# steineggerlab/unicore

Measured on AMD Instinct MI355X. Metric: 3Di alignments/sec (cluster path), higher is better.
Workload: dtype u16

## Files before the change

### include/unicore_cluster.h

```cpp
#ifndef UNICORE_CLUSTER_H
#define UNICORE_CLUSTER_H
#include <stddef.h>
#include <stdint.h>
#ifdef __cplusplus
extern "C" {
#endif

#define UC_OK 0
#define UC_ERR_GENERIC 1
#define UC_ERR_ARGS 2
#define UC_ERR_IO 3
#define UC_ERR_DEVICE 4

typedef struct uc_opts {
    uint32_t struct_size;
    int32_t threads;
    int32_t verbosity;
    int32_t device;
    int32_t num_gpus;
    const char *cluster_options;
    const char *data_dir;
} uc_opts;

#define UC_ABI_VERSION 9
// ... 94 lines not shown
int uc_hits_merge(uint32_t n_seqs, int32_t max_seqs, int n_parts, const uint32_t *const *counts,
                  const uc_hit *const *hits, uint32_t *out_counts, uc_hit *out_hits, uint64_t out_capacity,
                  uint64_t *out_n);

int uc_engine_hits_export_dev(const uc_engine *e, uint32_t *d_query, uint32_t *d_target, int32_t *d_score, int32_t *d_diag);
int uc_engine_hits_import_dev(uc_engine *e, uint64_t n, const uint32_t *d_query, const uint32_t *d_target, const int32_t *d_score,
                              const int32_t *d_diag, uint32_t rank, uint32_t world, uint64_t *n_kept);

typedef struct uc_comm uc_comm;
#define UC_COMM_ID_BYTES 128
int uc_comm_unique_id(uint8_t id[UC_COMM_ID_BYTES]);
int uc_comm_create(const uint8_t id[UC_COMM_ID_BYTES], int32_t rank, int32_t world, int32_t device, uc_comm **out);
void uc_comm_destroy(uc_comm *c);
int uc_comm_info(const uc_comm *c, int32_t *nccl_ranks, int32_t *nccl_rank, int32_t *device);
int uc_engine_cluster_step(uc_engine *e, uc_comm *comm, int32_t target_shards, uint32_t *assign, uint64_t *n_alignments);

int uc_engine_align(uc_engine *e, uint32_t qbegin, uint32_t qend);
int uc_engine_alns_get(const uc_engine *e, uint32_t qbegin, uint32_t qend, uc_aln *out);
int uc_engine_edges_size(const uc_engine *e, uint64_t *n_edges);
int uc_engine_edges_get(const uc_engine *e, uint32_t *edges );

int uc_engine_stats(const uc_engine *e, uc_stats *out);
void uc_engine_reset_stats(uc_engine *e);

int uc_setcover(uint32_t n, const uint32_t *edges, uint64_t n_edges, uint32_t *assign);
int uc_engine_setcover(uc_engine *e, const uint32_t *edges, uint64_t n_edges, uint32_t *assign);
int uc_cluster_graph(uint32_t n, const uint32_t *edges, uint64_t n_edges, const uint32_t *len, int32_t mode, uint32_t *assign);
int uc_engine_cluster_graph(uc_engine *e, int32_t mode, const uint32_t *edges, uint64_t n_edges, uint32_t *assign);
int uc_engine_reassign(uc_engine *e, const uint32_t *assign_in, uint32_t *assign_out, uint8_t *rejected_out, uint64_t counts[4]);
int uc_write_cluster_db(const char *out_cluster_db, uint32_t n, const uint32_t *assign);

int uc_engine_ungapped_batch(uc_engine *e, uint64_t n, const uint32_t *q, const uint32_t *t,
                             const int32_t *diag, int32_t *score_out);
int uc_engine_ungapped_all(uc_engine *e, uint32_t qbegin, uint32_t qend, uint32_t tbegin, uint32_t tend, uint64_t tile_bytes,
                           int32_t *score_out, int32_t *diag_out);
int uc_engine_sw_batch(uc_engine *e, int mode, uint64_t n, const uint32_t *q, const uint32_t *t,
                       const int32_t *qend_in, const int32_t *tend_in,
                       int32_t *score_out, int32_t *qend_out, int32_t *tend_out);
int uc_engine_sw_pass(uc_engine *e, int table, int mode, int band, int raw, uint64_t n, const uint32_t *q, const uint32_t *t,
                      const int32_t *box, const int32_t *known, int32_t *score_out, int32_t *qend_out, int32_t *tend_out,
                      int32_t *class_out, int32_t *aln_len_out, int32_t *idents_out, int32_t *gaps_out, int32_t *miss_out);
int uc_engine_sw_pass2(uc_engine *e, int table, int mode, int band, int raw, uint64_t n, const uint32_t *q, const uint32_t *t,
                       const int32_t *box, const int32_t *known, int32_t *score_out, int32_t *qend_out, int32_t *tend_out,
                       int32_t *class_out, int32_t *aln_len_out, int32_t *idents_out, int32_t *gaps_out, int32_t *miss_out,
                       int32_t *qend2_out, int32_t *tend2_out);

// ... 22 lines not shown
```

### unicore_amd/__init__.py

```python
import ctypes as C
import os

import numpy as np

_HERE = os.path.dirname(os.path.abspath(__file__))
LIB_PATH = os.path.join(_HERE, "libunicore_cluster.so")

UC_OK, UC_ERR_GENERIC, UC_ERR_ARGS, UC_ERR_IO, UC_ERR_DEVICE = 0, 1, 2, 3, 4
NSTAGE = 8
PHASES = ("prefilter", "exchange_lists_to_home", "merge_at_home", "exchange_pairs_to_owner", "install_owned", "gapped", "edge_gather", "rank0_serial_cover")
STAGES = ("load", "index", "kmer", "ungapped", "select", "gapped", "setcover", "output")


class UcOpts(C.Structure):
    _fields_ = [("struct_size", C.c_uint32), ("threads", C.c_int32), ("verbosity", C.c_int32), ("device", C.c_int32),
                ("num_gpus", C.c_int32), ("cluster_options", C.c_char_p), ("data_dir", C.c_char_p)]


class UcStats(C.Structure):
    _fields_ = [(n, C.c_uint64) for n in (
        "n_seqs", "n_residues", "n_index_entries", "n_sim_kmers", "n_kmer_hits", "n_candidates", "n_prefilter_hits",
        "n_gapped_alignments", "n_start_alignments", "n_pk_reruns", "n_edges", "n_clusters", "cells_fwd", "cells_rev", "cells_start")] + [
        ("algorithmic_bytes", C.c_uint64 * NSTAGE), ("stage_seconds", C.c_double * NSTAGE),
        ("sw_kernel_ms", C.c_double), ("sw_kernel_launches", C.c_uint64), ("sw_algorithmic_bytes", C.c_uint64),
# ... 11 lines not shown


class UcT5Stats(C.Structure):
    _fields_ = [("n_seqs", C.c_uint64), ("n_tokens", C.c_uint64), ("flops", C.c_double), ("gpu_ms", C.c_double),
                ("n_replicas", C.c_uint32), ("reserved0", C.c_uint32), ("gpu_ms_sum", C.c_double),
                ("tokens_min_replica", C.c_uint64), ("tokens_max_replica", C.c_uint64)]


HIT_DTYPE = np.dtype([("target", "<u4"), ("score", "<i4"), ("diag", "<i4")])
ALN_DTYPE = np.dtype([(n, "<i4") for n in ("score", "score_rev", "corrected", "qstart", "qend", "tstart", "tend",
                                            "aln_len", "idents", "pass_evalue", "accepted", "gap_opens")])

SYMBOLS = (
    "uc_cluster", "uc_createtsv", "uc_rmdb", "uc_search", "uc_convertalis", "uc_last_error", "uc_version", "uc_check_options",
    "uc_option_arity", "uc_release_scratch", "uc_createdb", "uc_t5_load", "uc_t5_free", "uc_t5_encode", "uc_t5_get_stats", "uc_comm_unique_id", "uc_comm_create", "uc_comm_destroy", "uc_comm_info", "uc_engine_cluster_step",
    "uc_engine_create", "uc_engine_destroy", "uc_engine_load_db", "uc_engine_set_db", "uc_engine_num_seqs",
    "uc_engine_prefilter", "uc_engine_prefilter_range", "uc_engine_hits_size", "uc_engine_hits_get", "uc_engine_hits_get_range", "uc_engine_hits_set", "uc_engine_hits_merge",
    "uc_engine_hits_export_dev", "uc_engine_hits_import_dev", "uc_engine_setcover",
    "uc_hits_merge", "uc_engine_align", "uc_engine_alns_get", "uc_engine_edges_size", "uc_engine_edges_get",
    "uc_engine_stats", "uc_engine_reset_stats", "uc_setcover", "uc_write_cluster_db",
    "uc_engine_ungapped_batch", "uc_engine_ungapped_all", "uc_engine_sw_batch", "uc_engine_sw_pass", "uc_engine_sw_pass2", "uc_engine_backtraces_size", "uc_engine_backtraces_get",
    "uc_backtrace_render", "uc_format_output_check", "uc_engine_tb_emit_pass", "uc_abi_version", "uc_stats_size", "uc_set_round_hook",
    "uc_t5_gemm_variant", "uc_t5_kernel_gemm", "uc_t5_kernel_rmsnorm", "uc_t5_kernel_attention", "uc_t5_kernel_cnn_head", "uc_t5_bias_table",
    "uc_cluster_graph", "uc_engine_cluster_graph", "uc_engine_reassign",
)
ABI_VERSION = 9
ROUND_HOOK = C.CFUNCTYPE(None, C.c_void_p, C.c_int32, C.c_uint32, C.POINTER(C.c_uint32), C.c_int32, C.c_void_p)

_lib = None


class UcError(RuntimeError):
    def __init__(self, code, msg):
        super().__init__("unicore_cluster error %d: %s" % (code, msg))
        self.code = code


def lib():
    global _lib
    if _lib is not None:
        return _lib
    if not os.path.exists(LIB_PATH):
        raise ImportError("%s is missing — run `make product` (or __graft_entry__.build()); there is no fallback path" % LIB_PATH)
    L = C.CDLL(LIB_PATH)
    vp, u32, u64, i32 = C.c_void_p, C.c_uint32, C.c_uint64, C.c_int32
    L.uc_last_error.restype = C.c_char_p
    L.uc_version.restype = C.c_char_p
# ... 22 lines not shown
    L.uc_engine_destroy.argtypes = [vp]
    L.uc_engine_destroy.restype = None
    L.uc_engine_load_db.argtypes = [vp, C.c_char_p]
    L.uc_engine_set_db.argtypes = [vp, u32, vp, vp, vp]
    L.uc_engine_num_seqs.argtypes = [vp]
    L.uc_engine_num_seqs.restype = u32
    L.uc_engine_prefilter.argtypes = [vp, u32, u32]
    L.uc_engine_hits_size.argtypes = [vp, C.POINTER(u64)]
    L.uc_engine_hits_get.argtypes = [vp, vp, vp]
    L.uc_engine_hits_get_range.argtypes = [vp, u32, u32, vp, vp]
    L.uc_engine_hits_set.argtypes = [vp, vp, vp]
    L.uc_engine_hits_merge.argtypes = [vp, C.c_int, C.POINTER(vp), C.POINTER(vp)]
    L.uc_engine_hits_export_dev.argtypes = [vp, vp, vp, vp, vp]
    L.uc_engine_setcover.argtypes = [vp, vp, u64, vp]
    L.uc_engine_hits_import_dev.argtypes = [vp, u64, vp, vp, vp, vp, u32, u32, C.POINTER(u64)]
    L.uc_hits_merge.argtypes = [u32, i32, C.c_int, C.POINTER(vp), C.POINTER(vp), vp, vp, u64, C.POINTER(u64)]
    L.uc_engine_align.argtypes = [vp, u32, u32]
    L.uc_engine_alns_get.argtypes = [vp, u32, u32, vp]
    L.uc_engine_edges_size.argtypes = [vp, C.POINTER(u64)]
    L.uc_engine_edges_get.argtypes = [vp, vp]
    L.uc_engine_stats.argtypes = [vp, C.POINTER(UcStats)]
    L.uc_engine_reset_stats.argtypes = [vp]
    L.uc_engine_reset_stats.restype = None
    L.uc_setcover.argtypes = [u32, vp, u64, vp]
    L.uc_cluster_graph.argtypes = [u32, vp, u64, vp, i32, vp]
    L.uc_engine_cluster_graph.argtypes = [vp, i32, vp, u64, vp]
    L.uc_engine_reassign.argtypes = [vp, vp, vp, vp, vp]
    L.uc_write_cluster_db.argtypes = [C.c_char_p, u32, vp]
    L.uc_engine_ungapped_batch.argtypes = [vp, u64, vp, vp, vp, vp]
    L.uc_engine_ungapped_all.argtypes = [vp, u32, u32, u32, u32, u64, vp, vp]
    L.uc_engine_sw_batch.argtypes = [vp, C.c_int, u64, vp, vp, vp, vp, vp, vp, vp]
    L.uc_engine_sw_pass.argtypes = [vp, C.c_int, C.c_int, C.c_int, C.c_int, u64, vp, vp, vp, vp] + [vp] * 8
    L.uc_engine_sw_pass2.argtypes = [vp, C.c_int, C.c_int, C.c_int, C.c_int, u64, vp, vp, vp, vp] + [vp] * 10
    L.uc_engine_backtraces_size.argtypes = [vp, u32, u32, C.POINTER(u64)]
    L.uc_engine_backtraces_get.argtypes = [vp, u32, u32, vp, vp]
    L.uc_backtrace_render.argtypes = [vp, u64, C.c_char_p, u64, C.POINTER(u64)]
    L.uc_format_output_check.argtypes = [C.c_char_p, C.POINTER(u32)]
    L.uc_engine_tb_emit_pass.argtypes = [vp, C.c_int, C.c_int, u64, vp, vp, vp, vp] + [vp] * 6 + [vp, vp, u64, C.POINTER(u64)]
    L.uc_t5_gemm_variant.argtypes = [i32, i32, i32, C.POINTER(i32)]
    L.uc_t5_kernel_gemm.argtypes = [i32, i32, i32, i32, i32, i32, vp, vp, vp]
    L.uc_t5_kernel_rmsnorm.argtypes = [i32, i32, i32, C.c_float, vp, vp, vp]
    L.uc_t5_kernel_attention.argtypes = [i32, i32, i32, vp, i32, vp, vp, vp]
    L.uc_t5_kernel_cnn_head.argtypes = [i32, i32, vp, i32, i32, i32, i32, i32, vp, vp, vp, vp, vp, vp, vp]
    L.uc_t5_bias_table.argtypes = [i32, i32, i32, i32, vp, vp]
    L.uc_abi_version.restype = u32
    L.uc_stats_size.restype = C.c_size_t
# ... 353 lines not shown
        k = C.c_uint64()
        _check(lib().uc_engine_cluster_step(self._h, comm._h if comm is not None else None, target_shards,
                                            assign.ctypes.data if rank0 else None, C.byref(k)))
        return assign, int(k.value)

    def alns(self, qbegin=0, qend=None):
        qend = self.n if qend is None else qend
        counts, _ = self.hits()
        n = int(counts[qbegin:qend].sum())
        out = np.zeros(max(n, 1), ALN_DTYPE)
        _check(lib().uc_engine_alns_get(self._h, qbegin, qend, out.ctypes.data))
        return out[:n]

    def edges(self):
        ne = C.c_uint64()
        _check(lib().uc_engine_edges_size(self._h, C.byref(ne)))
        e = np.zeros((max(ne.value, 1), 2), np.uint32)
        _check(lib().uc_engine_edges_get(self._h, e.ctypes.data))
        return e[: ne.value]

    def stats(self):
        st = UcStats()
        _check(lib().uc_engine_stats(self._h, C.byref(st)))
        return st.as_dict()

    def reset_stats(self):
        lib().uc_engine_reset_stats(self._h)

    def ungapped(self, q, t, diag):
        q = np.ascontiguousarray(q, np.uint32); t = np.ascontiguousarray(t, np.uint32)
        diag = np.ascontiguousarray(diag, np.int32)
        out = np.zeros(len(q), np.int32)
        _check(lib().uc_engine_ungapped_batch(self._h, len(q), q.ctypes.data, t.ctypes.data, diag.ctypes.data, out.ctypes.data))
        return out

    def ungapped_all(self, qbegin=0, qend=None, tbegin=0, tend=None, tile_bytes=0):
        qend = self.n if qend is None else qend
        tend = self.n if tend is None else tend
        score = np.zeros((max(qend - qbegin, 0), max(tend - tbegin, 0)), np.int32)
        diag = np.zeros_like(score)
        _check(lib().uc_engine_ungapped_all(self._h, qbegin, qend, tbegin, tend, tile_bytes, score.ctypes.data, diag.ctypes.data))
        return score, diag

    def sw(self, mode, q, t, qend=None, tend=None):
        q = np.ascontiguousarray(q, np.uint32); t = np.ascontiguousarray(t, np.uint32)
        n = len(q)
        qe = np.ascontiguousarray(qend, np.int32) if qend is not None else None
# ... 48 lines not shown
```

### unicore_amd/csrc/uc_capi.cpp

```cpp
#include <sys/stat.h>

#include <algorithm>
#include <cmath>
#include <cstdlib>
#include <cstring>
#include <fstream>
#include <future>
#include <memory>
#include <mutex>
#include <thread>

#include "uc_engine.h"
#include "uc_multi.h"
#include "uc_t5.h"

using namespace uc;

struct uc_engine {
    std::unique_ptr<Engine> e;
};
struct uc_comm {
    Comm c;
};
struct uc_t5 {
// ... 373 lines not shown

int uc_engine_edges_size(const uc_engine *e, uint64_t *n_edges) {
    return guard([&] { require(e, "engine"); require(n_edges, "n_edges"); *n_edges = e->e->edges_on_host ? e->e->edges.size() / 2 : e->e->n_edges_dev; });
}

int uc_engine_edges_get(const uc_engine *e, uint32_t *edges) {
    return guard([&] {
        require(e, "engine");
        const std::vector<uint32_t> &h = e->e->host_edges();
        if (!h.empty()) { require(edges, "edges"); memcpy(edges, h.data(), h.size() * 4); }
    });
}

int uc_engine_stats(const uc_engine *e, uc_stats *out) {
    return guard([&] { require(e, "engine"); require(out, "out"); *out = e->e->stats; });
}

void uc_engine_reset_stats(uc_engine *e) {
    if (!e || !e->e) return;
    uc_stats &s = e->e->stats;
    const uint64_t ns = s.n_seqs, nr = s.n_residues;
    memset(&s, 0, sizeof s);
    s.n_seqs = ns; s.n_residues = nr;
}

int uc_setcover(uint32_t n, const uint32_t *edges, uint64_t n_edges, uint32_t *assign) {
    return guard([&] {
        if (n) require(assign, "assign");
        if (n_edges) require(edges, "edges");
        set_cover(n, edges, n_edges, assign);
    });
}

int uc_engine_setcover(uc_engine *e, const uint32_t *edges, uint64_t n_edges, uint32_t *assign) {
    return guard([&] {
        require(e, "engine");
        const uint32_t n = e->e->hdb.n;
        if (n) require(assign, "assign");
        if (n_edges) require(edges, "edges");
        Timer tc;
        e->e->set_cover_device(n, edges, n_edges, assign);
        e->e->stats.stage_seconds[UC_ST_SETCOVER] += tc.seconds();
    });
}

int uc_cluster_graph(uint32_t n, const uint32_t *edges, uint64_t n_edges, const uint32_t *len, int32_t mode, uint32_t *assign) {
// ... 744 lines not shown
```

### unicore_amd/csrc/uc_engine.h

```cpp
#pragma once
#include <hip/hip_runtime.h>

#include <algorithm>
#include <atomic>
#include <chrono>
#include <cstdint>
#include <cstdio>
#include <cstdlib>
#include <mutex>
#include <string>
#include <utility>
#include <vector>

#include "uc_common.h"
#include "uc_db.h"
#include "uc_device.h"
#include "uc_options.h"
#include "unicore_cluster.h"

namespace uc {

struct OomRelief { bool (*fn)(void *) = nullptr; void *ctx = nullptr; };
inline OomRelief &oom_relief_slot() { static thread_local OomRelief r; return r; }
inline bool oom_test_fires() {
// ... 198 lines not shown
    DevBuf<uint32_t> d_bt_runs, d_bt_n;
    DevBuf<unsigned long long> d_bt_pos;
    uint64_t bt_used = 0;
    void get_backtraces(uint64_t begin, uint64_t n, uint64_t *run_off, std::vector<uint32_t> &runs) const;
    DevBuf<uint32_t> d_edges;
    uint64_t n_edges_dev = 0;
    std::vector<uint32_t> edges;
    bool edges_on_host = true;
    void clear_edges() { edges.clear(); n_edges_dev = 0; edges_on_host = true; }
    const std::vector<uint32_t> &host_edges();

    uc_stats stats{};

    explicit Engine(const Params &pp, int dev);
    ~Engine();
    void upload_db(bool keep_raw = false);
    void upload_sub_db(const std::vector<uint32_t> &cur, const std::vector<uint64_t> &full_off);
    uint64_t plan_db_layout();
    void finish_db_install(struct Timer &tm);
    void prefilter(uint32_t tbegin, uint32_t tend, uint32_t qbegin = 0, uint32_t qend = UINT32_MAX);
    void prefilter_cells(uint32_t tbegin, uint32_t tend, const std::vector<std::pair<uint32_t, uint32_t>> &others);
    PrefilterScratch *pre = nullptr;
    AlignScratch *aln = nullptr;
    uint64_t last_align_hits = 0;
    void drop_scratch();
    bool relieve_pressure(int stage);
    int stage_frames[3] = {0, 0, 0};
    struct PressureScope {
        OomRelief saved;
        struct Ctx { Engine *e; int stage; } ctx;
        PressureScope(Engine &E, int stage) : saved(oom_relief_slot()), ctx{&E, stage} {
            E.stage_frames[stage]++;
            oom_relief_slot() = OomRelief{[](void *c) { return ((Ctx *)c)->e->relieve_pressure(((Ctx *)c)->stage); }, &ctx};
        }
        ~PressureScope() { oom_relief_slot() = saved; ctx.e->stage_frames[ctx.stage]--; }
        PressureScope(const PressureScope &) = delete;
        PressureScope &operator=(const PressureScope &) = delete;
    };
    uint64_t prefilter_chunk_residues = 96ull << 20;
    void set_hits(const uint32_t *counts, const uc_hit *h, bool check_max_seqs = true);
    void get_hits(uc_hit *out) const;
    void get_hits_range(uint64_t begin, uint64_t k, uc_hit *out) const;
    void export_hits_dev(uint32_t *dq, uint32_t *dt, int32_t *ds, int32_t *dd) const;
    uint64_t import_hits_dev(uint64_t n, const uint32_t *dq, const uint32_t *dt, const int32_t *ds, const int32_t *dd,
                             uint32_t rank, uint32_t world);
    uint64_t merge_hits_dev(uint64_t n1, const uint32_t *q1, const uint32_t *t1, const int32_t *s1, const int32_t *d1,
// ... 38 lines not shown
```

### unicore_amd/csrc/uc_prefilter.hip

```cpp
#include <hip/hip_runtime.h>

#include <algorithm>
#include <cstdlib>
#include <cstring>
#include <type_traits>

#include <rocprim/rocprim.hpp>

#include "uc_engine.h"

namespace uc {

constexpr uint32_t KMER_INVALID = 0xFFFFFFFFu;

struct KmerCfg {
    int koff[K];
    int span;
    int thr;
};

__device__ __forceinline__ uint32_t find_seq(const uint32_t *off, uint32_t lo, uint32_t hi, uint32_t p) {
    while (hi - lo > 1) {
        const uint32_t mid = lo + ((hi - lo) >> 1);
        if (off[mid] <= p) lo = mid; else hi = mid;
// ... 1016 lines not shown
                }
                if (nin < 64) break;
            }
            if (carry) {
                const uint64_t d = carry_key & dmask, a = (carry_cnt << 32) | (0xFFFFFFFFull - d), c2 = (carry_cnt << 32) | d;
                b1 = a > b1 ? a : b1; b2 = c2 > b2 ? c2 : b2;
            }
            if ((int)(b1 >> 32) >= min_hits) {
                const uint32_t gq = qbegin + (uint32_t)(grp >> fmt.tbits), gt = (uint32_t)(grp & tmask);
                const bool mir = gq >= mirror_q0;
                if (lane == 0) {
                    s_q[wv][staged] = gq; s_t[wv][staged] = gt; s_d[wv][staged] = (int)(0xFFFFFFFFull - (b1 & 0xFFFFFFFFull)) - fmt.dbias;
                    if (mir) { s_q[wv][staged + 1] = gt; s_t[wv][staged + 1] = gq; s_d[wv][staged + 1] = -((int)(b2 & 0xFFFFFFFFull) - fmt.dbias); }
                }
                staged += mir ? 2u : 1u;
                __builtin_amdgcn_wave_barrier();
                if (staged >= 64) drain();
            }
        }
    }
    if (staged) drain();
}

__global__ void __launch_bounds__(256) select_key_kernel(uint64_t n, const uint32_t *cq, const uint32_t *ct, const int32_t *score,
                                                         int min_score, uint64_t *key, unsigned long long *n_kept) {
    unsigned long long kept = 0;
    for (uint64_t i = (uint64_t)blockIdx.x * 256 + threadIdx.x; i < n; i += (uint64_t)gridDim.x * 256) {
        const int s = score[i];
        const bool ok = s >= min_score;
        key[i] = ok ? ((uint64_t)cq[i] << 32) | ((uint64_t)(255 - s) << 24) | ct[i] : ~0ull;
        kept += ok;
    }
    for (int o = 32; o > 0; o >>= 1) kept += __shfl_down(kept, o, 64);
    if ((threadIdx.x & 63) == 0 && kept) atomicAdd(n_kept, kept);
}

__global__ void __launch_bounds__(256) rank_flag_kernel(const uint64_t *skey, uint64_t n, uint32_t max_seqs, uint32_t *flag) {
    for (uint64_t i = (uint64_t)blockIdx.x * 256 + threadIdx.x; i < n; i += (uint64_t)gridDim.x * 256) {
        const uint64_t qk = skey[i] & 0xFFFFFFFF00000000ull;
        flag[i] = (i < max_seqs || skey[i - max_seqs] < qk) ? 1u : 0u;
    }
}

__global__ void __launch_bounds__(256) hit_scatter_kernel(const uint64_t *skey, const int32_t *sdiag, uint64_t n, const uint32_t *flag,
                                                          const uint64_t *pos, uint32_t *hq, uint32_t *ht, int32_t *hs, int32_t *hd) {
    for (uint64_t i = (uint64_t)blockIdx.x * 256 + threadIdx.x; i < n; i += (uint64_t)gridDim.x * 256) {
// ... 47 lines not shown
            const unsigned long long m = __ballot(o == w);
            if (m && (threadIdx.x & 63) == (unsigned)__ffsll((long long)m) - 1) atomicAdd(count + w, (unsigned long long)__popcll(m));
        }
    }
}
__global__ void __launch_bounds__(256) owner_gather_kernel(uint64_t n, const uint32_t *idx, const uint32_t *hq, const uint32_t *ht, const int32_t *hs,
                                                           const int32_t *hd, uint32_t *oq, uint32_t *ot, int32_t *os, int32_t *od) {
    for (uint64_t i = (uint64_t)blockIdx.x * 256 + threadIdx.x; i < n; i += (uint64_t)gridDim.x * 256) {
        const uint32_t j = idx[i];
        oq[i] = hq[j]; ot[i] = ht[j]; os[i] = hs[j]; od[i] = hd[j];
    }
}

struct WidenU32 {
    __host__ __device__ uint64_t operator()(uint32_t x) const { return (uint64_t)x; }
};

struct PrefilterScratch {
    DevBuf<unsigned long long> d_counters;
    DevBuf<char> d_temp;
    DevBuf<uint32_t> d_koff, k_in, k_out, d_ent32, v_in32, d_okey, d_okey2, d_oidx, d_order;
    DevBuf<uint64_t> d_ent, v_in;
    DevBuf<uint32_t> d_cnt, d_flag, d_cq, d_ct, d_rpidx2, d_qsurv;
    DevBuf<uint64_t> d_keys, d_keys2, d_pos, d_skey, d_skey2, d_rval2, d_qbase, d_soff, d_qr;
    DevBuf<int32_t> d_cd, d_cd2, d_score, d_mval;
    DevBuf<uint64_t> d_mkey;
    DevBuf<uint32_t> acc_q, acc_t, pass_q, pass_t;
    DevBuf<int32_t> acc_s, acc_d, pass_s, pass_d;
    DevBuf<uint8_t> d_kflag, d_wflag;
    DevBuf<uint32_t> d_qk, d_kid, d_dk, d_nsimk, d_drk, d_drk2, d_roff, d_nr, d_src, d_ph;
    DevBuf<uint64_t> d_drv, d_drv2, d_cumh, d_cumr, d_qh, d_qrn;
    DevBuf<RankRec> d_rec;
    DevBuf<uint32_t> d_kbits;
    UngappedAllWork ua;
    template <class F> void each(F f) {
        f(d_counters); f(d_temp); f(d_koff); f(k_in); f(k_out); f(d_ent32); f(v_in32); f(d_okey); f(d_okey2); f(d_oidx); f(d_order);
        f(d_ent); f(v_in); f(d_cnt); f(d_flag); f(d_cq); f(d_ct); f(d_rpidx2); f(d_qsurv); f(d_keys); f(d_keys2); f(d_pos); f(d_skey);
        f(d_skey2); f(d_rval2); f(d_qbase); f(d_soff); f(d_qr); f(d_cd); f(d_cd2); f(d_score); f(d_kflag); f(d_wflag); f(d_qk); f(d_kid); f(d_dk);
        f(d_nsimk); f(d_drk); f(d_drk2); f(d_roff); f(d_nr); f(d_src); f(d_ph); f(d_drv); f(d_drv2); f(d_cumh); f(d_cumr); f(d_qh); f(d_qrn); f(d_rec); f(d_kbits); f(d_mkey); f(d_mval); f(acc_q); f(acc_t); f(pass_q); f(pass_t); f(acc_s); f(acc_d); f(pass_s); f(pass_d);
        f(ua.score); f(ua.diag); f(ua.pairs); f(ua.prof); f(ua.prof_off);
    }
    size_t bytes() {
        size_t b = 0;
        each([&](auto &x) { b += x.cap * sizeof(*x.p); });
        return b;
    }
    void release_bytes(size_t target) {
        if (getenv("UC_TIMING")) {
            fprintf(stderr, "unicore-cluster[timing]: prefilter scratch %.1f GiB, %.1f GiB to give back before the gapped stage; buffers >= 2 GiB (index in PrefilterScratch::each: GiB):", bytes() / 1073741824.0, target / 1073741824.0);
            int i = 0;
            each([&](auto &x) { const double g = x.cap * sizeof(*x.p) / 1073741824.0; if (g >= 2.0) fprintf(stderr, " %d:%.1f", i, g); i++; });
            fprintf(stderr, "\n");
        }
        if (!target) return;
        if (target >= bytes()) { each([&](auto &x) { if (x.cap * sizeof(*x.p) >= ((size_t)1 << 30)) x.release(); }); return; }
        size_t freed = 0;
        while (freed < target) {
            size_t best = 0;
            each([&](auto &x) { best = std::max(best, x.cap * sizeof(*x.p)); });
            if (best < ((size_t)256 << 20)) break;
            bool done = false;
            each([&](auto &x) { if (!done && x.cap * sizeof(*x.p) == best) { x.release(); done = true; } });
            freed += best;
// ... 29 lines not shown
    const uint32_t n = hdb.n;
    if (n_hits) {
        pre->d_cnt.reserve(n);
        hipLaunchKernelGGL(hit_count_kernel, grid_for(n), dim3(256), 0, stream, d_hq.p, n_hits, n, pre->d_cnt.p);
        UC_HIP(hipMemcpyAsync(hit_cnt.data(), pre->d_cnt.p, (size_t)n * 4, hipMemcpyDeviceToHost, stream));
        UC_HIP(hipStreamSynchronize(stream));
    }
    for (uint32_t q = 0; q < n; q++) hit_off[q + 1] = hit_off[q] + hit_cnt[q];
    if (hit_off[n] != n_hits) fail(UC_ERR_GENERIC, "%s: hit list bookkeeping mismatch", who);
}

constexpr uint64_t RUN_MAX = 1ull << 29;
struct PrefilterPass {
    KmerCfg cfg;
    KeyFmt fmt;
    uint32_t tbegin = 0, tend = 0;
    uint32_t qbegin = 0, qend = 0;
    uint32_t mirror_q0 = UINT32_MAX;
    bool count_sims = false;
    double density_limit = 0.0, *density_out = nullptr;
    const void *ent_p = nullptr;
    uint32_t n_entries = 0;
    uint64_t HIT_CAP = 0, HIT_CAP_BIG = 0, DRUN_MAX = 0;
    uint64_t n_hits_total = 0, n_cand_total = 0, cand_cap = 0, run_cap = 1ull << 20;
    double t_kmer = 0, t_ung = 0, t_sel = 0, gpu_ms = 0;
};
struct SuperBatch {
    uint32_t begin = 0, end = 0;
    uint32_t P0 = 0, NP = 0;
    std::vector<uint64_t> h_qh, h_qr;
    uint64_t hit_cap = 0;
    double frac = 1.0;
};
struct QueryBatch {
    uint32_t qa = 0, qb = 0;
    uint64_t total_hits = 0, n_runs = 0;
    uint32_t qp0 = 0, qp1 = 0, nq_res = 0;
    unsigned kbits = 0;
    const uint64_t *sorted = nullptr;
    uint64_t n_sort = 0;
};
static KeyFmt key_format(const Engine &E, uint32_t tbegin, uint32_t tend) {
    KeyFmt fmt;
    const uint32_t m = std::min<uint32_t>(std::max<uint32_t>(E.max_len, 2), 65536u);
    fmt.dbits = 1;
    while ((1u << (fmt.dbits - 1)) < m) fmt.dbits++;
    fmt.dbias = 1 << (fmt.dbits - 1);
    fmt.tbits = 1;
    while ((1u << fmt.tbits) < E.hdb.n) fmt.tbits++;
    int rbits = 1;
    while ((1ull << rbits) < (uint64_t)std::max<uint32_t>(tend - tbegin, 1)) rbits++;
    fmt.compact = rbits + fmt.dbits <= 32 && !getenv("UC_PREFILTER_WIDE");
    fmt.tbase = tbegin;
    return fmt;
}

static void build_index(Engine &E, PrefilterPass &PP) {
    PrefilterScratch &S = *E.pre;
    Timer t_index;
    E.timed_ms_begin();
    const uint32_t tp0 = E.h_poff[PP.tbegin], tp1 = E.h_poff[PP.tend];
    const uint32_t nres = tp1 - tp0;
    S.d_koff.reserve((size_t)KSPACE + 1);
// ... 190 lines not shown
    return lp + lc;
}

static void expand_keys_filtered(Engine &E, PrefilterPass &PP, QueryBatch &B) {
    PrefilterScratch &S = *E.pre;
    const KeyFmt &fmt = PP.fmt;
    const uint32_t qa = B.qa, qp0 = B.qp0, nq = B.qb - B.qa;
    S.d_qbase.reserve(nq); S.d_qsurv.reserve(nq); S.d_soff.reserve((size_t)nq + 1);
    const uint64_t region_cap = B.total_hits + (uint64_t)KPT * nq;
    S.d_keys.reserve(fmt.compact ? region_cap : 2 * region_cap);
    S.d_qr.reserve((size_t)nq + 1);
    hipLaunchKernelGGL(run_range_kernel, grid_for((uint64_t)nq + 1), dim3(256), 0, E.stream, E.ddb, qa, nq, qp0, S.d_rpidx2.p, B.n_runs, S.d_qr.p);
    S.d_okey.reserve(nq); S.d_okey2.reserve(nq); S.d_oidx.reserve(nq); S.d_order.reserve(nq);
    hipLaunchKernelGGL(run_order_key_kernel, grid_for(nq), dim3(256), 0, E.stream, nq, S.d_qr.p, S.d_okey.p, S.d_oidx.p);
    rocprim_call(S.d_temp, [&](void *t, size_t &b) { return rocprim::radix_sort_pairs(t, b, S.d_okey.p, S.d_okey2.p, S.d_oidx.p, S.d_order.p, (size_t)nq, 0u, 32u, E.stream); });
    auto launch = [&](auto kern) {
        static PerDeviceOnce once[2];
        once[fmt.compact ? 1 : 0]([&] { UC_HIP(hipFuncSetAttribute((const void *)kern, hipFuncAttributeMaxDynamicSharedMemorySize, (int)filter_lds(FILTER_RPT))); });
        hipLaunchKernelGGL(kern, dim3(nq), dim3(FT), filter_lds(FILTER_RPT), E.stream, E.ddb, qa, qp0, S.d_rpidx2.p, S.d_rval2.p, S.d_qr.p, S.d_order.p, PP.ent_p, fmt,
                           S.d_counters.p + 5, (void *)S.d_keys.p, region_cap, S.d_qbase.p, S.d_qsurv.p);
    };
    if (fmt.compact) launch(filter_kernel<true>);
    else launch(filter_kernel<false>);
    const uint64_t n_sort = compact_u64(E, S.d_temp, S.d_qsurv.p, S.d_soff.p, nq);
    if (n_sort) {
        S.d_keys2.reserve(2 * n_sort);
        hipLaunchKernelGGL(fmt.compact ? compact_kernel<true> : compact_kernel<false>, dim3(std::min<uint32_t>(nq, 65535u)), dim3(256), 0, E.stream,
                           (const void *)S.d_keys.p, S.d_qbase.p, S.d_qsurv.p, S.d_soff.p, nq, fmt, S.d_keys2.p);
        rocprim_call(S.d_temp, [&](void *t, size_t &b) { return rocprim::radix_sort_keys(t, b, S.d_keys2.p, S.d_keys2.p + n_sort, (size_t)n_sort, 0u, B.kbits, E.stream); });
    }
    B.sorted = S.d_keys2.p + n_sort; B.n_sort = n_sort;
    E.stats.n_filtered_hits += n_sort;
}

static void expand_keys_plain(Engine &E, PrefilterPass &PP, QueryBatch &B) {
    PrefilterScratch &S = *E.pre;
    S.d_keys.reserve(B.total_hits); S.d_keys2.reserve(B.total_hits);
    const RunList rl{S.d_rpidx2.p, S.d_rval2.p, PP.run_cap};
    hipLaunchKernelGGL(expand_kernel, grid_for(B.n_runs), dim3(256), 0, E.stream, E.ddb, B.qa, B.qb, B.qp0, rl, B.n_runs, PP.ent_p, PP.fmt,
                       S.d_counters.p + 5, S.d_keys.p, B.total_hits);
    rocprim_call(S.d_temp, [&](void *t, size_t &b) { return rocprim::radix_sort_keys(t, b, S.d_keys.p, S.d_keys2.p, (size_t)B.total_hits, 0u, B.kbits, E.stream); });
    B.sorted = S.d_keys2.p; B.n_sort = B.total_hits;
    E.stats.n_filtered_hits += B.n_sort;
}

static uint64_t select_diagonals(Engine &E, PrefilterPass &PP, const QueryBatch &B) {
    PrefilterScratch &S = *E.pre;
    PP.cand_cap = std::max<uint64_t>(PP.cand_cap, std::max<uint64_t>(1u << 20, B.total_hits / 32));
    for (;;) {
        S.d_cq.reserve(PP.cand_cap); S.d_ct.reserve(PP.cand_cap); S.d_cd.reserve(PP.cand_cap);
        UC_HIP(hipMemsetAsync(S.d_counters.p + 6, 0, 8, E.stream));
        if (B.n_sort) {
            S.d_wflag.reserve((B.n_sort + 63) / 64 + 64);
            hipLaunchKernelGGL(diag_select_kernel, grid_for(B.n_sort), dim3(256), 0, E.stream, B.sorted, B.n_sort, E.p.min_diag_hits, PP.fmt, B.qa,
                               S.d_counters.p + 6, PP.cand_cap, S.d_cq.p, S.d_ct.p, S.d_cd.p, PP.mirror_q0, S.d_wflag.p);
            hipLaunchKernelGGL(diag_long_kernel, grid_for((B.n_sort + 63) / 64), dim3(256), 0, E.stream, B.sorted, B.n_sort, E.p.min_diag_hits, PP.fmt, B.qa,
                               S.d_counters.p + 6, PP.cand_cap, S.d_cq.p, S.d_ct.p, S.d_cd.p, PP.mirror_q0, (const uint8_t *)S.d_wflag.p);
        }
        unsigned long long nc = 0;
        UC_HIP(hipMemcpyAsync(&nc, S.d_counters.p + 6, 8, hipMemcpyDeviceToHost, E.stream));
        UC_HIP(hipStreamSynchronize(E.stream));
        if (nc <= PP.cand_cap) return nc;
        PP.cand_cap = nc;
    }
}

static void rescore_ungapped(Engine &E, PrefilterPass &PP, uint64_t n_cand) {
    PrefilterScratch &S = *E.pre;
    Timer t_u;
    E.timed_ms_begin();
    S.d_score.reserve(n_cand);
    launch_ungapped(E.ddb, n_cand, S.d_cq.p, S.d_ct.p, S.d_cd.p, S.d_score.p, S.d_counters.p + 2, E.stream);
    UC_HIP(hipGetLastError());
    PP.gpu_ms += E.timed_ms_end();
    PP.t_ung += t_u.seconds();
}

static void select_and_append(Engine &E, PrefilterPass &PP, uint64_t n_cand) {
    PrefilterScratch &S = *E.pre;
    Timer t_s;
    E.timed_ms_begin();
    S.d_skey.reserve(n_cand); S.d_skey2.reserve(n_cand); S.d_cd2.reserve(n_cand);
    UC_HIP(hipMemsetAsync(S.d_counters.p + 1, 0, 8, E.stream));
    hipLaunchKernelGGL(select_key_kernel, grid_for(n_cand), dim3(256), 0, E.stream, n_cand, S.d_cq.p, S.d_ct.p, S.d_score.p, E.p.min_ungapped, S.d_skey.p, S.d_counters.p + 1);
    rocprim_call(S.d_temp, [&](void *t, size_t &b) { return rocprim::radix_sort_pairs(t, b, S.d_skey.p, S.d_skey2.p, S.d_cd.p, S.d_cd2.p, (size_t)n_cand, 0u, 64u, E.stream); });
    unsigned long long kept = 0;
    UC_HIP(hipMemcpyAsync(&kept, S.d_counters.p + 1, 8, hipMemcpyDeviceToHost, E.stream));
    UC_HIP(hipStreamSynchronize(E.stream));
    if (kept) {
        S.d_flag.reserve(kept); S.d_pos.reserve(kept);
        hipLaunchKernelGGL(rank_flag_kernel, grid_for(kept), dim3(256), 0, E.stream, S.d_skey2.p, (uint64_t)kept, (uint32_t)E.p.max_seqs, S.d_flag.p);
        const uint64_t add = compact_u64(E, S.d_temp, S.d_flag.p, S.d_pos.p, kept), n_hits = E.n_hits;
        E.d_hq.grow_preserve(n_hits + add, n_hits, E.stream); E.d_ht.grow_preserve(n_hits + add, n_hits, E.stream);
        E.d_hs.grow_preserve(n_hits + add, n_hits, E.stream); E.d_hd.grow_preserve(n_hits + add, n_hits, E.stream);
        hipLaunchKernelGGL(hit_scatter_kernel, grid_for(kept), dim3(256), 0, E.stream, S.d_skey2.p, S.d_cd2.p, (uint64_t)kept, S.d_flag.p, S.d_pos.p,
                           E.d_hq.p + n_hits, E.d_ht.p + n_hits, E.d_hs.p + n_hits, E.d_hd.p + n_hits);
        E.n_hits += add;
    }
    UC_HIP(hipGetLastError());
    PP.gpu_ms += E.timed_ms_end();
    PP.t_sel += t_s.seconds();
}

static void finish_chunk(Engine &E, const PrefilterPass &PP, uint64_t sims_before) {
    if (PP.mirror_q0 == UINT32_MAX) E.finish_hit_lists("prefilter");
    uc_stats &stats = E.stats;
    unsigned long long ovl = 0;
    UC_HIP(hipMemcpy(&ovl, E.pre->d_counters.p + 2, 8, hipMemcpyDeviceToHost));
    stats.n_kmer_hits += PP.n_hits_total;
    stats.n_candidates += PP.n_cand_total;
    stats.algorithmic_bytes[UC_ST_KMER] += 8ull * (stats.n_sim_kmers - sims_before) + 6ull * PP.n_hits_total + 8ull * PP.n_cand_total;
    stats.algorithmic_bytes[UC_ST_UNGAPPED] += ovl + 16ull * PP.n_cand_total;
    stats.algorithmic_bytes[UC_ST_SELECT] += 16ull * PP.n_cand_total;
    stats.stage_seconds[UC_ST_KMER] += PP.t_kmer;
    stats.stage_seconds[UC_ST_UNGAPPED] += PP.t_ung;
    stats.stage_seconds[UC_ST_SELECT] += PP.t_sel;
    stats.prefilter_kernel_ms += PP.gpu_ms;
}

static bool prefilter_one(Engine &E, uint32_t tbegin, uint32_t tend, uint32_t qbegin, uint32_t qend, bool count_sims, double density_limit,
                          double *density_out, uint32_t mirror_q0) {
    UC_HIP(hipSetDevice(E.device));
    const uint32_t n = E.hdb.n;
    PrefilterPass PP;
    for (int m = 0; m < K; m++) PP.cfg.koff[m] = E.p.koff[m];
    PP.cfg.span = E.p.span; PP.cfg.thr = E.p.kmer_thr;
    PP.tbegin = tbegin; PP.tend = tend; PP.qbegin = qbegin; PP.qend = qend; PP.mirror_q0 = mirror_q0;
    PP.count_sims = count_sims; PP.density_limit = density_limit; PP.density_out = density_out;
    const char *hc = getenv("UC_HIT_CAP");
    PP.HIT_CAP = hc ? std::max<uint64_t>(1u << 20, strtoull(hc, nullptr, 10)) : (3ull << 29);
    PP.HIT_CAP_BIG = hc ? PP.HIT_CAP : (15ull << 28);
    const char *dm = getenv("UC_DRUN_MAX");
    PP.DRUN_MAX = dm ? std::max<uint64_t>(1, strtoull(dm, nullptr, 10)) : (1ull << 31);

    E.hit_cnt.assign(n, 0);
    E.hit_off.assign((size_t)n + 1, 0);
    E.n_hits = 0;
    E.alns_valid = false;
    E.clear_edges();
    const uint64_t sims_before = E.stats.n_sim_kmers;

    if (n > (1u << 24)) fail(UC_ERR_GENERIC, "prefilter: %u sequences exceed the 2^24 limit of the hit keys", n);
    if (!E.pre) E.pre = ParkedScratch<PrefilterScratch>::take_or_new(E.device);
    E.pre->d_counters.reserve(8);
    UC_HIP(hipMemsetAsync(E.pre->d_counters.p, 0, 64, E.stream));

    build_index(E, PP);
    SuperBatch SB;
    SB.begin = SB.end = qbegin;
    for (uint32_t qa = qbegin; qa < qend;) {
        if (qa >= SB.end && !choose_superbatch(E, PP, SB, qa)) return false;
        Timer t_b;
        E.timed_ms_begin();
        QueryBatch B = cut_batch(E, PP, SB, qa);
        uint64_t n_cand = 0;
        if (B.total_hits) {
// ... 287 lines not shown
```

Measured before the change: 22.40 million.

## Select diagonal candidates on-chip per query with block radix sort

Adds a per-query block kernel that sorts each query's surviving target/diagonal keys in shared memory with rocprim block_radix_sort. It then finds the best diagonal per target and writes candidates straight back, so small queries skip the global compact, radix sort and expand path. A gather kernel appends these candidates after the globally processed ones, and the select-stage pair sort now uses fewer key bits based on the sequence count. This adds extra kernel launches (one block per query, with early exits), counters and a stats API, and it depends on the caps and the mirror handling being correct.

```diff
diff --git a/include/unicore_cluster.h b/include/unicore_cluster.h
--- a/include/unicore_cluster.h
+++ b/include/unicore_cluster.h
@@ -140,6 +140,7 @@
 
 int uc_engine_stats(const uc_engine *e, uc_stats *out);
 void uc_engine_reset_stats(uc_engine *e);
+int uc_engine_td_onchip(const uc_engine *e, uint64_t *out );
 
 int uc_setcover(uint32_t n, const uint32_t *edges, uint64_t n_edges, uint32_t *assign);
 int uc_engine_setcover(uc_engine *e, const uint32_t *edges, uint64_t n_edges, uint32_t *assign);
diff --git a/unicore_amd/__init__.py b/unicore_amd/__init__.py
--- a/unicore_amd/__init__.py
+++ b/unicore_amd/__init__.py
@@ -57,7 +57,7 @@
     "uc_engine_ungapped_batch", "uc_engine_ungapped_all", "uc_engine_sw_batch", "uc_engine_sw_pass", "uc_engine_sw_pass2", "uc_engine_backtraces_size", "uc_engine_backtraces_get",
     "uc_backtrace_render", "uc_format_output_check", "uc_engine_tb_emit_pass", "uc_abi_version", "uc_stats_size", "uc_set_round_hook",
     "uc_t5_gemm_variant", "uc_t5_kernel_gemm", "uc_t5_kernel_rmsnorm", "uc_t5_kernel_attention", "uc_t5_kernel_cnn_head", "uc_t5_bias_table",
-    "uc_cluster_graph", "uc_engine_cluster_graph", "uc_engine_reassign",
+    "uc_cluster_graph", "uc_engine_cluster_graph", "uc_engine_reassign", "uc_engine_td_onchip",
 )
 ABI_VERSION = 9
 ROUND_HOOK = C.CFUNCTYPE(None, C.c_void_p, C.c_int32, C.c_uint32, C.POINTER(C.c_uint32), C.c_int32, C.c_void_p)
@@ -126,6 +126,7 @@
     L.uc_engine_stats.argtypes = [vp, C.POINTER(UcStats)]
     L.uc_engine_reset_stats.argtypes = [vp]
     L.uc_engine_reset_stats.restype = None
+    L.uc_engine_td_onchip.argtypes = [vp, C.POINTER(C.c_uint64)]
     L.uc_setcover.argtypes = [u32, vp, u64, vp]
     L.uc_cluster_graph.argtypes = [u32, vp, u64, vp, i32, vp]
     L.uc_engine_cluster_graph.argtypes = [vp, i32, vp, u64, vp]
@@ -525,7 +526,11 @@
     def stats(self):
         st = UcStats()
         _check(lib().uc_engine_stats(self._h, C.byref(st)))
-        return st.as_dict()
+        d = st.as_dict()
+        td = (C.c_uint64 * 4)()
+        _check(lib().uc_engine_td_onchip(self._h, td))
+        d["td_onchip_queries"], d["td_onchip_keys"] = int(td[0]), int(td[2])
+        return d
 
     def reset_stats(self):
         lib().uc_engine_reset_stats(self._h)
diff --git a/unicore_amd/csrc/uc_capi.cpp b/unicore_amd/csrc/uc_capi.cpp
--- a/unicore_amd/csrc/uc_capi.cpp
+++ b/unicore_amd/csrc/uc_capi.cpp
@@ -419,6 +419,11 @@
     const uint64_t ns = s.n_seqs, nr = s.n_residues;
     memset(&s, 0, sizeof s);
     s.n_seqs = ns; s.n_residues = nr;
+    for (uint64_t &x : e->e->td_onchip) x = 0;
+}
+
+int uc_engine_td_onchip(const uc_engine *e, uint64_t *out) {
+    return guard([&] { require(e, "engine"); require(out, "out"); for (int i = 0; i < 4; i++) out[i] = e->e->td_onchip[i]; });
 }
 
 int uc_setcover(uint32_t n, const uint32_t *edges, uint64_t n_edges, uint32_t *assign) {
diff --git a/unicore_amd/csrc/uc_engine.h b/unicore_amd/csrc/uc_engine.h
--- a/unicore_amd/csrc/uc_engine.h
+++ b/unicore_amd/csrc/uc_engine.h
@@ -244,6 +244,7 @@
     void prefilter_cells(uint32_t tbegin, uint32_t tend, const std::vector<std::pair<uint32_t, uint32_t>> &others);
     PrefilterScratch *pre = nullptr;
     AlignScratch *aln = nullptr;
+    uint64_t td_onchip[4] = {0, 0, 0, 0};
     uint64_t last_align_hits = 0;
     void drop_scratch();
     bool relieve_pressure(int stage);
diff --git a/unicore_amd/csrc/uc_prefilter.hip b/unicore_amd/csrc/uc_prefilter.hip
--- a/unicore_amd/csrc/uc_prefilter.hip
+++ b/unicore_amd/csrc/uc_prefilter.hip
@@ -1062,6 +1062,176 @@
     if (staged) drain();
 }
 
+constexpr int TDS_T = 256;
+constexpr int TDS_MAX_IPT = 32;
+constexpr uint32_t TDS_CAP = TDS_T * TDS_MAX_IPT;
+template <int IPT> using TdSort = rocprim::block_radix_sort<uint32_t, TDS_T, IPT>;
+constexpr size_t tds_max(size_t a, size_t b) { return a > b ? a : b; }
+constexpr int TDS_SMALL_IPT = 8;
+constexpr size_t TDS_SORT_BYTES_SMALL =
+    tds_max(tds_max(sizeof(TdSort<1>::storage_type), sizeof(TdSort<2>::storage_type)), tds_max(sizeof(TdSort<4>::storage_type), sizeof(TdSort<8>::storage_type)));
+constexpr size_t TDS_SORT_BYTES_BIG = tds_max(sizeof(TdSort<16>::storage_type), sizeof(TdSort<32>::storage_type));
+
+struct TdsMax { template <class T> __device__ T operator()(T a, T b) const { return a > b ? a : b; } };
+struct TdsSum { template <class T> __device__ T operator()(T a, T b) const { return a + b; } };
+template <class T, class Op>
+__device__ __forceinline__ T tds_block_excl(T v, Op op, T *s_w, T *total) {
+    const int lane = threadIdx.x & 63, wv = threadIdx.x >> 6;
+    T inc = v;
+    for (int o = 1; o < 64; o <<= 1) {
+        const T u = (T)__shfl_up((unsigned long long)inc, o, 64);
+        if (lane >= o) inc = op(u, inc);
+    }
+    if (lane == 63) s_w[wv] = inc;
+    __syncthreads();
+    T ex = (T)__shfl_up((unsigned long long)inc, 1, 64), all = 0;
+    if (lane == 0) ex = 0;
+    for (int w = 0; w < TDS_T / 64; w++) {
+        const T u = s_w[w];
+        if (w < wv) ex = op(u, ex);
+        all = op(all, u);
+    }
+    __syncthreads();
+    if (total) *total = all;
+    return ex;
+}
+
+__device__ __forceinline__ void tds_block_excl_max2(uint64_t a, uint64_t b, uint64_t *s_w, uint64_t &ea, uint64_t &eb) {
+    const int lane = threadIdx.x & 63, wv = threadIdx.x >> 6;
+    for (int o = 1; o < 64; o <<= 1) {
+        const uint64_t ua = (uint64_t)__shfl_up((unsigned long long)a, o, 64), ub = (uint64_t)__shfl_up((unsigned long long)b, o, 64);
+        if (lane >= o) { a = ua > a ? ua : a; b = ub > b ? ub : b; }
+    }
+    if (lane == 63) { s_w[2 * wv] = a; s_w[2 * wv + 1] = b; }
+    __syncthreads();
+    ea = (uint64_t)__shfl_up((unsigned long long)a, 1, 64); eb = (uint64_t)__shfl_up((unsigned long long)b, 1, 64);
+    if (lane == 0) ea = eb = 0;
+    for (int w = 0; w < wv; w++) {
+        const uint64_t ua = s_w[2 * w], ub = s_w[2 * w + 1];
+        ea = ua > ea ? ua : ea; eb = ub > eb ? ub : eb;
+    }
+    __syncthreads();
+}
+
+template <int IPT>
+__device__ __forceinline__ uint32_t td_select_sorted(uint32_t *reg, uint32_t n, int min_hits, int dbits, unsigned end_bit, bool mirror, void *s_sort,
+                                                     uint32_t (*s_edge)[TDS_T], uint64_t *s_w) {
+    const int tid = threadIdx.x;
+    const uint32_t dmask = (1u << dbits) - 1u;
+    uint32_t keys[IPT];
+#pragma unroll
+    for (int j = 0; j < IPT; j++) {
+        const uint32_t i = (uint32_t)j * TDS_T + tid;
+        keys[j] = i < n ? reg[i] : 0xFFFFFFFFu;
+    }
+    TdSort<IPT>().sort(keys, *reinterpret_cast<typename TdSort<IPT>::storage_type *>(s_sort), 0u, end_bit);
+    const uint32_t i0 = (uint32_t)tid * IPT;
+    s_edge[0][tid] = keys[0]; s_edge[1][tid] = keys[IPT - 1];
+    __syncthreads();
+    const uint32_t kprev = tid ? s_edge[1][tid - 1] : 0u, knext = tid < TDS_T - 1 ? s_edge[0][tid + 1] : 0u;
+    __syncthreads();
+    uint32_t rs = 0;
+    uint64_t m1 = 0, m2 = 0;
+    auto step = [&](int j) -> bool {
+        const uint32_t i = i0 + (uint32_t)j, k = keys[j];
+        const uint32_t kp = j ? keys[j ? j - 1 : 0] : kprev, kn = j < IPT - 1 ? keys[j < IPT - 1 ? j + 1 : j] : knext;
+        if (i >= n) return false;
+        if (i == 0 || kp != k) rs = i;
+        const bool last = i == n - 1;
+        if (last || kn != k) {
+            const uint64_t g = ((uint64_t)(k >> dbits) << 32) | ((uint64_t)(i + 1 - rs) << dbits);
+            const uint64_t a = g | (uint64_t)(dmask - (k & dmask)), b = g | (uint64_t)(k & dmask);
+            m1 = a > m1 ? a : m1; m2 = b > m2 ? b : m2;
+        }
+        return last || (kn >> dbits) != (k >> dbits);
+    };
+#pragma unroll
+    for (int j = 0; j < IPT; j++) {
+        const uint32_t i = i0 + (uint32_t)j, kp = j ? keys[j ? j - 1 : 0] : kprev;
+        if (i < n && (i == 0 || kp != keys[j])) rs = i;
+    }
+    const uint32_t rs0 = (uint32_t)tds_block_excl<uint64_t>((uint64_t)rs, TdsMax(), s_w, nullptr);
+    rs = rs0;
+#pragma unroll
+    for (int j = 0; j < IPT; j++) (void)step(j);
+    uint64_t e1, e2;
+    tds_block_excl_max2(m1, m2, s_w, e1, e2);
+    uint32_t mine = 0;
+    rs = rs0; m1 = e1; m2 = e2;
+#pragma unroll
+    for (int j = 0; j < IPT; j++)
+        if (step(j)) mine += (int)((uint32_t)m1 >> dbits) >= min_hits ? 1u : 0u;
+    uint64_t tot64 = 0;
+    uint32_t w = (uint32_t)tds_block_excl<uint64_t>((uint64_t)mine, TdsSum(), s_w, &tot64);
+    const uint32_t ncand = (uint32_t)tot64;
+    if (mine) {
+        rs = rs0; m1 = e1; m2 = e2;
+#pragma unroll
+        for (int j = 0; j < IPT; j++)
+            if (step(j) && (int)((uint32_t)m1 >> dbits) >= min_hits) {
+                const uint32_t g = (keys[j] >> dbits) << dbits;
+                reg[w] = g | (dmask - ((uint32_t)m1 & dmask));
+                if (mirror) reg[ncand + w] = g | ((uint32_t)m2 & dmask);
+                w++;
+            }
+    }
+    return ncand;
+}
+
+template <bool BIG>
+__global__ void __launch_bounds__(TDS_T) td_select_kernel(uint32_t *region, const uint64_t *qbase, uint32_t *qsurv, const uint32_t *order, uint32_t qbegin,
+                                                          uint32_t mirror_q0, int min_hits, int dbits, unsigned end_bit, uint32_t cap,
+                                                          uint32_t *qcand, uint32_t *qmir, uint32_t *qrec, unsigned long long *n_taken) {
+    __shared__ __attribute__((aligned(16))) char s_sort[BIG ? TDS_SORT_BYTES_BIG : TDS_SORT_BYTES_SMALL];
+    __shared__ uint32_t s_edge[2][TDS_T];
+    __shared__ uint64_t s_w[2 * TDS_T / 64];
+    constexpr uint32_t SMALL = (uint32_t)TDS_SMALL_IPT * TDS_T;
+    const uint32_t qi = order[blockIdx.x];
+    const uint32_t n = qsurv[qi];
+    if (n == 0 || n > cap) {
+        if (!BIG && threadIdx.x == 0) { qcand[qi] = 0; qmir[qi] = 0; qrec[qi] = 0; }
+        return;
+    }
+    if (BIG != (n > SMALL)) return;
+    uint32_t *reg = region + qbase[qi];
+    const bool mirror = mirror_q0 != UINT32_MAX && qbegin + qi >= mirror_q0;
+    uint32_t nc;
+    if (BIG) {
+        if (n <= 16u * TDS_T) nc = td_select_sorted<16>(reg, n, min_hits, dbits, end_bit, mirror, s_sort, s_edge, s_w);
+        else nc = td_select_sorted<32>(reg, n, min_hits, dbits, end_bit, mirror, s_sort, s_edge, s_w);
+    } else {
+        if (n <= 1u * TDS_T) nc = td_select_sorted<1>(reg, n, min_hits, dbits, end_bit, mirror, s_sort, s_edge, s_w);
+        else if (n <= 2u * TDS_T) nc = td_select_sorted<2>(reg, n, min_hits, dbits, end_bit, mirror, s_sort, s_edge, s_w);
+        else if (n <= 4u * TDS_T) nc = td_select_sorted<4>(reg, n, min_hits, dbits, end_bit, mirror, s_sort, s_edge, s_w);
+        else nc = td_select_sorted<8>(reg, n, min_hits, dbits, end_bit, mirror, s_sort, s_edge, s_w);
+    }
+    if (threadIdx.x == 0) {
+        qcand[qi] = nc; qmir[qi] = mirror ? nc : 0u; qrec[qi] = mirror ? 2u * nc : nc;
+        qsurv[qi] = 0;
+        atomicAdd(n_taken, (1ull << 40) | (unsigned long long)n);
+    }
+}
+
+__global__ void __launch_bounds__(256) cand_gather_kernel(const uint32_t *region, const uint64_t *qbase, const uint32_t *qcand, const uint32_t *qmir,
+                                                          const uint64_t *coff, uint32_t nq, KeyFmt fmt, uint32_t qbegin, uint64_t out0,
+                                                          uint32_t *cq, uint32_t *ct, int32_t *cd) {
+    const int lane = threadIdx.x & 63, wv = threadIdx.x >> 6;
+    const uint32_t dmask = (1u << fmt.dbits) - 1u;
+    for (uint32_t qi = blockIdx.x * 4 + wv; qi < nq; qi += gridDim.x * 4) {
+        const uint32_t nc = qcand[qi], nr = nc + qmir[qi];
+        if (!nr) continue;
+        const uint64_t src = qbase[qi], dst = out0 + coff[qi];
+        const uint32_t q = qbegin + qi;
+        for (uint32_t k = lane; k < nr; k += 64) {
+            const uint32_t td = region[src + k];
+            const uint32_t t = (td >> fmt.dbits) + fmt.tbase;
+            const int32_t d = (int32_t)(td & dmask) - fmt.dbias;
+            const bool plain = k < nc;
+            cq[dst + k] = plain ? q : t; ct[dst + k] = plain ? t : q; cd[dst + k] = plain ? d : -d;
+        }
+    }
+}
+
 __global__ void __launch_bounds__(256) select_key_kernel(uint64_t n, const uint32_t *cq, const uint32_t *ct, const int32_t *score,
                                                          int min_score, uint64_t *key, unsigned long long *n_kept) {
     unsigned long long kept = 0;
@@ -1155,6 +1325,8 @@
     DevBuf<uint32_t> d_koff, k_in, k_out, d_ent32, v_in32, d_okey, d_okey2, d_oidx, d_order;
     DevBuf<uint64_t> d_ent, v_in;
     DevBuf<uint32_t> d_cnt, d_flag, d_cq, d_ct, d_rpidx2, d_qsurv;
+    DevBuf<uint32_t> d_qcand, d_qmir, d_qrec;
+    DevBuf<uint64_t> d_coff;
     DevBuf<uint64_t> d_keys, d_keys2, d_pos, d_skey, d_skey2, d_rval2, d_qbase, d_soff, d_qr;
     DevBuf<int32_t> d_cd, d_cd2, d_score, d_mval;
     DevBuf<uint64_t> d_mkey;
@@ -1171,7 +1343,7 @@
         f(d_ent); f(v_in); f(d_cnt); f(d_flag); f(d_cq); f(d_ct); f(d_rpidx2); f(d_qsurv); f(d_keys); f(d_keys2); f(d_pos); f(d_skey);
         f(d_skey2); f(d_rval2); f(d_qbase); f(d_soff); f(d_qr); f(d_cd); f(d_cd2); f(d_score); f(d_kflag); f(d_wflag); f(d_qk); f(d_kid); f(d_dk);
         f(d_nsimk); f(d_drk); f(d_drk2); f(d_roff); f(d_nr); f(d_src); f(d_ph); f(d_drv); f(d_drv2); f(d_cumh); f(d_cumr); f(d_qh); f(d_qrn); f(d_rec); f(d_kbits); f(d_mkey); f(d_mval); f(acc_q); f(acc_t); f(pass_q); f(pass_t); f(acc_s); f(acc_d); f(pass_s); f(pass_d);
-        f(ua.score); f(ua.diag); f(ua.pairs); f(ua.prof); f(ua.prof_off);
+        f(d_qcand); f(d_qmir); f(d_qrec); f(d_coff); f(ua.score); f(ua.diag); f(ua.pairs); f(ua.prof); f(ua.prof_off);
     }
     size_t bytes() {
         size_t b = 0;
@@ -1247,6 +1419,8 @@
     const void *ent_p = nullptr;
     uint32_t n_entries = 0;
     uint64_t HIT_CAP = 0, HIT_CAP_BIG = 0, DRUN_MAX = 0;
+    uint64_t td_queries = 0, td_keys = 0, filt_queries = 0, filt_keys = 0;
+    uint32_t td_cap = 0;
     uint64_t n_hits_total = 0, n_cand_total = 0, cand_cap = 0, run_cap = 1ull << 20;
     double t_kmer = 0, t_ung = 0, t_sel = 0, gpu_ms = 0;
 };
@@ -1264,6 +1438,7 @@
     unsigned kbits = 0;
     const uint64_t *sorted = nullptr;
     uint64_t n_sort = 0;
+    uint64_t n_rec = 0;
 };
 static KeyFmt key_format(const Engine &E, uint32_t tbegin, uint32_t tend) {
     KeyFmt fmt;
@@ -1500,7 +1675,29 @@
     };
     if (fmt.compact) launch(filter_kernel<true>);
     else launch(filter_kernel<false>);
-    const uint64_t n_sort = compact_u64(E, S.d_temp, S.d_qsurv.p, S.d_soff.p, nq);
+    unsigned long long taken = 0;
+    uint32_t last_rec = 0;
+    const bool onchip = fmt.compact && PP.td_cap > 0;
+    if (onchip) {
+        int rbits = 1;
+        while ((1ull << rbits) < (uint64_t)std::max<uint32_t>(PP.tend - PP.tbegin, 1)) rbits++;
+        S.d_qcand.reserve(nq); S.d_qmir.reserve(nq); S.d_qrec.reserve(nq); S.d_coff.reserve(nq);
+        UC_HIP(hipMemsetAsync(S.d_counters.p + 7, 0, 8, E.stream));
+        hipLaunchKernelGGL(td_select_kernel<false>, dim3(nq), dim3(TDS_T), 0, E.stream, (uint32_t *)S.d_keys.p, S.d_qbase.p, S.d_qsurv.p, S.d_order.p, qa, PP.mirror_q0,
+                           E.p.min_diag_hits, fmt.dbits, (unsigned)std::min(32, rbits + fmt.dbits), PP.td_cap, S.d_qcand.p, S.d_qmir.p, S.d_qrec.p, S.d_counters.p + 7);
+        if (PP.td_cap > (uint32_t)TDS_SMALL_IPT * TDS_T)
+            hipLaunchKernelGGL(td_select_kernel<true>, dim3(nq), dim3(TDS_T), 0, E.stream, (uint32_t *)S.d_keys.p, S.d_qbase.p, S.d_qsurv.p, S.d_order.p, qa, PP.mirror_q0,
+                               E.p.min_diag_hits, fmt.dbits, (unsigned)std::min(32, rbits + fmt.dbits), PP.td_cap, S.d_qcand.p, S.d_qmir.p, S.d_qrec.p, S.d_counters.p + 7);
+        auto rin = rocprim::make_transform_iterator(S.d_qrec.p, WidenU32());
+        rocprim_call(S.d_temp, [&](void *t, size_t &b) { return rocprim::exclusive_scan(t, b, rin, S.d_coff.p, (uint64_t)0, (size_t)nq, rocprim::plus<uint64_t>(), E.stream); });
+        UC_HIP(hipMemcpyAsync(&B.n_rec, S.d_coff.p + (nq - 1), 8, hipMemcpyDeviceToHost, E.stream));
+        UC_HIP(hipMemcpyAsync(&taken, S.d_counters.p + 7, 8, hipMemcpyDeviceToHost, E.stream));
+    }
+    const uint64_t n_sort = compact_u64(E, S.d_temp, S.d_qsurv.p, S.d_soff.p, nq, onchip ? S.d_qrec.p + (nq - 1) : nullptr, &last_rec);
+    B.n_rec += last_rec;
+    const uint64_t taken_keys = taken & ((1ull << 40) - 1);
+    PP.td_queries += taken >> 40; PP.td_keys += taken_keys; PP.filt_queries += nq; PP.filt_keys += n_sort + taken_keys;
+    E.td_onchip[0] += taken >> 40; E.td_onchip[1] += nq; E.td_onchip[2] += taken_keys; E.td_onchip[3] += n_sort + taken_keys;
     if (n_sort) {
         S.d_keys2.reserve(2 * n_sort);
         hipLaunchKernelGGL(fmt.compact ? compact_kernel<true> : compact_kernel<false>, dim3(std::min<uint32_t>(nq, 65535u)), dim3(256), 0, E.stream,
@@ -1508,7 +1705,7 @@
         rocprim_call(S.d_temp, [&](void *t, size_t &b) { return rocprim::radix_sort_keys(t, b, S.d_keys2.p, S.d_keys2.p + n_sort, (size_t)n_sort, 0u, B.kbits, E.stream); });
     }
     B.sorted = S.d_keys2.p + n_sort; B.n_sort = n_sort;
-    E.stats.n_filtered_hits += n_sort;
+    E.stats.n_filtered_hits += n_sort + taken_keys;
 }
 
 static void expand_keys_plain(Engine &E, PrefilterPass &PP, QueryBatch &B) {
@@ -1526,7 +1723,7 @@
     PrefilterScratch &S = *E.pre;
     PP.cand_cap = std::max<uint64_t>(PP.cand_cap, std::max<uint64_t>(1u << 20, B.total_hits / 32));
     for (;;) {
-        S.d_cq.reserve(PP.cand_cap); S.d_ct.reserve(PP.cand_cap); S.d_cd.reserve(PP.cand_cap);
+        S.d_cq.reserve(PP.cand_cap + B.n_rec); S.d_ct.reserve(PP.cand_cap + B.n_rec); S.d_cd.reserve(PP.cand_cap + B.n_rec);
         UC_HIP(hipMemsetAsync(S.d_counters.p + 6, 0, 8, E.stream));
         if (B.n_sort) {
             S.d_wflag.reserve((B.n_sort + 63) / 64 + 64);
@@ -1538,7 +1735,12 @@
         unsigned long long nc = 0;
         UC_HIP(hipMemcpyAsync(&nc, S.d_counters.p + 6, 8, hipMemcpyDeviceToHost, E.stream));
         UC_HIP(hipStreamSynchronize(E.stream));
-        if (nc <= PP.cand_cap) return nc;
+        if (nc <= PP.cand_cap) {
+            if (B.n_rec)
+                hipLaunchKernelGGL(cand_gather_kernel, grid_for((uint64_t)(B.qb - B.qa) * 64), dim3(256), 0, E.stream, (const uint32_t *)S.d_keys.p, S.d_qbase.p,
+                                   S.d_qcand.p, S.d_qmir.p, S.d_coff.p, B.qb - B.qa, PP.fmt, B.qa, (uint64_t)nc, S.d_cq.p, S.d_ct.p, S.d_cd.p);
+            return nc + B.n_rec;
+        }
         PP.cand_cap = nc;
     }
 }
@@ -1561,7 +1763,9 @@
     S.d_skey.reserve(n_cand); S.d_skey2.reserve(n_cand); S.d_cd2.reserve(n_cand);
     UC_HIP(hipMemsetAsync(S.d_counters.p + 1, 0, 8, E.stream));
     hipLaunchKernelGGL(select_key_kernel, grid_for(n_cand), dim3(256), 0, E.stream, n_cand, S.d_cq.p, S.d_ct.p, S.d_score.p, E.p.min_ungapped, S.d_skey.p, S.d_counters.p + 1);
-    rocprim_call(S.d_temp, [&](void *t, size_t &b) { return rocprim::radix_sort_pairs(t, b, S.d_skey.p, S.d_skey2.p, S.d_cd.p, S.d_cd2.p, (size_t)n_cand, 0u, 64u, E.stream); });
+    unsigned kb = 33;
+    while (kb < 64 && (1ull << (kb - 32)) <= E.hdb.n) kb++;
+    rocprim_call(S.d_temp, [&](void *t, size_t &b) { return rocprim::radix_sort_pairs(t, b, S.d_skey.p, S.d_skey2.p, S.d_cd.p, S.d_cd2.p, (size_t)n_cand, 0u, kb, E.stream); });
     unsigned long long kept = 0;
     UC_HIP(hipMemcpyAsync(&kept, S.d_counters.p + 1, 8, hipMemcpyDeviceToHost, E.stream));
     UC_HIP(hipStreamSynchronize(E.stream));
@@ -1582,6 +1786,9 @@
 
 static void finish_chunk(Engine &E, const PrefilterPass &PP, uint64_t sims_before) {
     if (PP.mirror_q0 == UINT32_MAX) E.finish_hit_lists("prefilter");
+    if (getenv("UC_TIMING") && PP.filt_queries)
+        fprintf(stderr, "unicore-cluster[timing]: on-chip diagonal selection (cap %u): %llu of %llu queries, %llu of %llu surviving keys\n", PP.td_cap,
+                (unsigned long long)PP.td_queries, (unsigned long long)PP.filt_queries, (unsigned long long)PP.td_keys, (unsigned long long)PP.filt_keys);
     uc_stats &stats = E.stats;
     unsigned long long ovl = 0;
     UC_HIP(hipMemcpy(&ovl, E.pre->d_counters.p + 2, 8, hipMemcpyDeviceToHost));
@@ -1610,6 +1817,14 @@
     PP.HIT_CAP_BIG = hc ? PP.HIT_CAP : (15ull << 28);
     const char *dm = getenv("UC_DRUN_MAX");
     PP.DRUN_MAX = dm ? std::max<uint64_t>(1, strtoull(dm, nullptr, 10)) : (1ull << 31);
+    const char *to = getenv("UC_TD_ONCHIP"), *tc = getenv("UC_TD_ONCHIP_CAP");
+    PP.td_cap = to && atoi(to) == 0 ? 0u : TDS_CAP;
+    if (PP.td_cap && tc) {
+        const uint64_t want = strtoull(tc, nullptr, 10);
+        uint32_t c = 64;
+        while (c < TDS_CAP && 2ull * c <= want) c *= 2;
+        PP.td_cap = c;
+    }
 
     E.hit_cnt.assign(n, 0);
     E.hit_off.assign((size_t)n + 1, 0);
```

Result: faster. 22.65 million, median of 6 (+1.1%).
